# zhai-lw/L3AC

Measured on AMD Instinct MI355X. Metric: audio samples/sec encode+decode, 1kbps@16kHz, batch 256; indices bit-exact, higher is better.
Workload: dtype f32

## Files before the change

l3ac_amd/csrc/capi.hip:

```cpp
#include <algorithm>
#include <cmath>
#include <cstdarg>
#include <cstdlib>
#include <cstring>
#include <new>
#include <string>
#include <vector>

#include "network.hpp"
#include "kernels/split_bf16.hpp"

static thread_local std::string g_last_error;

void l3ac_set_error(const char* fmt, ...) {
    char buf[1024];
    va_list ap;
    va_start(ap, fmt);
    vsnprintf(buf, sizeof(buf), fmt, ap);
    va_end(ap);
    g_last_error = buf;
}

int l3ac_device_cu_count() {
    static std::atomic<int> cus[L3AC_MAX_DEVICES] = {};
// ... 97 lines not shown
template <class Map>
auto lookup(const Map& m, const char* name, const char* kind) -> decltype(m.begin()->second) {
    if (!name) {
        l3ac_set_error("null block name");
        return nullptr;
    }
    auto it = m.find(name);
    if (it == m.end()) {
        l3ac_set_error("no %s block named '%s'", kind, name);
        return nullptr;
    }
    return it->second;
}

struct Option {
    const char* name;
    int& (*field)(l3ac_ctx&);
    bool flag;
    int lo, hi, def;
    const char* env;
};
#define L3AC_FIELD(member) [](l3ac_ctx& c) -> int& { return c.member; }
const Option kOptions[] = {
    {"gemm_split", L3AC_FIELD(gemm_split), true, 0, 1, 1, "L3AC_GEMM_SPLIT"},
    {"head_pretanh", L3AC_FIELD(head_pretanh), true, 0, 1, 0, nullptr},
    {"narrow_ring", L3AC_FIELD(narrow_ring), false, 0, 2, 1, nullptr},
    {"wide_sliced", L3AC_FIELD(wide_sliced), false, 0, 2, 1, nullptr},
    {"unit_counter", L3AC_FIELD(unit_counter), false, 0, 3, 1, "L3AC_UNIT_COUNTER"},
    {"trans_coop", L3AC_FIELD(coop.enabled), true, 0, 1, 1, "L3AC_TRANS_COOP"},
    {"coop_timeout_ms", L3AC_FIELD(coop.timeout_ms), false, 1, 20000, 250, nullptr},
    {"down_fused", L3AC_FIELD(down_fused), false, 0, 2, 2, "L3AC_DOWN_FUSED"},
    {"gemm_w256", L3AC_FIELD(gemm_w256), false, 0, 2, 1, "L3AC_GEMM_W256"},
    {"unit_chunk_mb", L3AC_FIELD(unit_chunk_mb), false, 0, 65536, 192, "L3AC_UNIT_CHUNK_MB"},
};
#undef L3AC_FIELD

const Option* find_option(const char* name) {
    for (const Option& o : kOptions)
        if (std::strcmp(o.name, name) == 0) return &o;
    return nullptr;
}

int unknown_option(const char* who, const char* name) {
    std::string names;
    for (const Option& o : kOptions) names += std::string(names.empty() ? "" : ", ") + o.name;
    l3ac_set_error("%s: unknown option '%s' (%s; to set only: coop_release_claim, coop_test_fault)", who, name, names.c_str());
    return L3AC_EINVAL;
}

int initial_value(const Option& o) {
    const char* e = o.env ? std::getenv(o.env) : nullptr;
    return e ? std::atoi(e) : o.def;
}

int checked_value(const Option& o, int value) { return o.flag ? value != 0 : std::min(std::max(value, o.lo), o.hi); }

int set_checked(l3ac_ctx* ctx, const Option& o, int value, const char* who) {
    L3AC_REQUIRE(!(std::strcmp(o.name, "down_fused") == 0 && value == 1),
                 "%s: down_fused = 1 (the bf16x3 one-kernel down layers) was retired, DESIGN.md section 4; 2 (the default) is the one-kernel "
                 "form with the bits of 0, the GEMM + row kernel", who);
    o.field(*ctx) = checked_value(o, value);
    return L3AC_OK;
}

int ragged_plan(l3ac_ctx* ctx, hipStream_t s, RaggedPlan& p, int batch, int max_tok, const int32_t* n_tok, const int32_t* samples) {
    p.max_tok = max_tok;
// ... 282 lines not shown
                    const float* w_out, const float* b_out, float* q_feature, void* stream) {
    L3AC_REQUIRE(indices && levels && n_levels >= 1 && n_levels <= L3AC_MAX_LEVELS, "fsq_decode: bad arguments");
    FsqArgs f{};
    f.idx_in = indices; f.n = n; f.feat = feat; f.n_levels = n_levels;
    for (int d = 0; d < n_levels; ++d) f.levels[d] = levels[d];
    f.w_out = w_out; f.b_out = b_out; f.q_feature = q_feature;
    return launch_fsq((hipStream_t)stream, f);
}

int l3ac_fsq_copy_ceiling(const float* x, int64_t n, float* q_feature, int32_t* indices, float* level_indices, void* stream) {
    return launch_fsq_copy_ceiling((hipStream_t)stream, x, n, q_feature, indices, level_indices);
}
int l3ac_fsq_copy_ceiling_at(const float* x, int64_t n, float* q_feature, int32_t* indices, float* level_indices, int32_t blocks_per_cu, void* stream) {
    return launch_fsq_copy_ceiling((hipStream_t)stream, x, n, q_feature, indices, level_indices, blocks_per_cu);
}

int64_t l3ac_vq_argmin_scratch_bytes(int64_t n, int32_t k, int32_t form) {
    return (n > 0 && k > 0) ? (int64_t)vq_argmin_scratch_bytes(n, k, form) : 0;
}

int l3ac_vq_argmin(const float* queries, int64_t n, const float* codebook, int32_t k, int32_t dim, int32_t* out_idx,
                   void* scratch, int64_t scratch_bytes, int32_t form, void* stream) {
    L3AC_REQUIRE(queries && codebook && out_idx, "vq_argmin: null buffer");
    if (n == 0) return L3AC_OK;
    L3AC_REQUIRE(form == 0 || form == 1, "vq_argmin: form must be 0 (automatic) or 1 (direct-form scan)");
    L3AC_REQUIRE(scratch && k > 0 && scratch_bytes >= (int64_t)vq_argmin_scratch_bytes(n, k, form),
                 "vq_argmin: scratch of %lld bytes needed (l3ac_vq_argmin_scratch_bytes), %lld given",
                 (long long)(k > 0 ? vq_argmin_scratch_bytes(n, k, form) : 0), (long long)scratch_bytes);
    return launch_vq_argmin((hipStream_t)stream, queries, n, codebook, k, dim, scratch, out_idx, form);
}

int l3ac_op_first_block(l3ac_ctx* ctx, const float* audio, int32_t batch, int32_t samples, float* y, void* stream) {
    L3AC_ENTER_WS(ctx, stream);
    return launch_first_block((hipStream_t)stream, ctx->first, audio, samples, batch, samples, samples, y);
}

int l3ac_op_first_block_at(l3ac_ctx* ctx, const float* audio, int32_t batch, int32_t samples, int64_t audio_stride, int32_t frames,
                           float* y, void* stream) {
    L3AC_ENTER_WS(ctx, stream);
    L3AC_REQUIRE(audio && y && batch > 0, "op_first_block_at: bad arguments");
    L3AC_REQUIRE(samples > 0 && frames >= samples, "op_first_block_at: frames %d < samples %d, or samples <= 0", frames, samples);
    L3AC_REQUIRE(audio_stride >= samples, "op_first_block_at: stride %lld < samples %d", (long long)audio_stride, samples);
    return launch_first_block((hipStream_t)stream, ctx->first, audio, audio_stride, batch, samples, frames, y);
}

static int op_shape_ok(int batch, int frames) {
    L3AC_REQUIRE(frames <= L3AC_MAX_CLIP_FRAMES, "block entry: %d frames per clip, the limit is 2^31 - 65536 (32-bit frame numbers)", frames);
    L3AC_REQUIRE((int64_t)batch * frames < L3AC_MAX_ROWS, "block entry: batch * frames = %lld, the limit is 2^34 rows (32-bit tile numbers)",
                 (long long)batch * frames);
    return L3AC_OK;
}

#define L3AC_OP_SCRATCH(c_max)                                                                                    \
    L3AC_TRY(op_shape_ok(batch, frames));                                                                         \
    L3AC_TRY(workspace_ensure(ctx, (size_t)batch * frames * (c_max), (size_t)batch * frames * (c_max),           \
                              std::max((size_t)batch * frames * 4 * (c_max),                                      \
                                       (conv_unit_wide_scratch_bytes((c_max), (int64_t)batch * frames) + 3) / 4), \
                              (size_t)batch * frames * 4, (size_t)batch, (hipStream_t)stream))

int l3ac_op_conv_unit(l3ac_ctx* ctx, const char* block, const float* x, int32_t batch, int32_t frames, float* y,
                      void* stream) {
    L3AC_ENTER_WS(ctx, stream);
    const ConvUnitW* w = lookup(ctx->by_unit, block, "ConvUnit");
    if (!w) return L3AC_EINVAL;
    L3AC_TRY(conv_unit_shape_ok(ctx, *w, x == y, frames));
    L3AC_OP_SCRATCH(w->c);
    return run_conv_unit(ctx, (hipStream_t)stream, *w, x, y, batch, frames);
}

int l3ac_op_down_layer(l3ac_ctx* ctx, const char* block, const float* x, int32_t batch, int32_t frames, float* y,
                       void* stream) {
    L3AC_ENTER_WS(ctx, stream);
    const DownW* w = lookup(ctx->by_down, block, "down-layer");
    if (!w) return L3AC_EINVAL;
    L3AC_REQUIRE(x != y, "op_down_layer: x and y must not alias");
    return run_down(ctx, (hipStream_t)stream, *w, x, y, batch, frames);
// ... 165 lines not shown
        out[slot].ms_total += ms;
        out[slot].flops += r.flops;
        out[slot].bytes += r.bytes;
    }
    if (p->failed && rc == L3AC_OK) {
        l3ac_set_error("profile: event creation failed");
        rc = L3AC_EHIP;
    }
    delete p;
    if (n_out) *n_out = n;
    return rc;
}

int l3ac_gemm_f32(const float* a, int64_t lda, const float* w, const float* bias, float* c, int64_t ldc, int64_t m,
                  int32_t n, int32_t k, void* stream) {
    GemmArgs g{};
    g.a = a; g.lda = lda; g.w = w; g.ldw = k; g.c = c; g.ldc = ldc; g.m = m; g.n = n; g.k = k; g.bias = bias; g.epi = EPI_BIAS;
    return launch_gemm((hipStream_t)stream, g);
}

void l3ac_split3_host(const float* x, int64_t n, uint16_t* planes) {
    for (int64_t i = 0; i < n; ++i) {
        uint16_t pl[3];
        split3_host(x[i], pl);
        planes[i] = pl[0];
        planes[n + i] = pl[1];
        planes[2 * n + i] = pl[2];
    }
}

int l3ac_ctx_set_head_pretanh(l3ac_ctx* ctx, int32_t enable) { return l3ac_ctx_set_option(ctx, "head_pretanh", enable); }

int l3ac_op_snake(const float* x, float* y, int64_t rows, int32_t c, const float* alpha, int32_t mode, void* stream) {
    L3AC_REQUIRE(x && y && alpha && rows >= 0 && c > 0 && c % 4 == 0 && c <= 4096 && mode >= 0 && mode <= 4, "op_snake: bad arguments");
    hipStream_t s = (hipStream_t)stream;
    float* inv = nullptr;
    std::vector<float> ha((size_t)c), hi((size_t)c);
    L3AC_HIP_CHECK(hipMemcpyAsync(ha.data(), alpha, (size_t)c * sizeof(float), hipMemcpyDeviceToHost, s));
    L3AC_HIP_CHECK(hipStreamSynchronize(s));
    for (int i = 0; i < c; ++i) hi[i] = 1.0f / (ha[i] + 1e-8f);
    L3AC_HIP_CHECK(hipMalloc((void**)&inv, (size_t)c * sizeof(float)));
    int rc = L3AC_OK;
    if (hipMemcpyAsync(inv, hi.data(), (size_t)c * sizeof(float), hipMemcpyHostToDevice, s) != hipSuccess) {
        l3ac_set_error("op_snake: upload failed");
        rc = L3AC_EHIP;
    }
    if (rc == L3AC_OK) rc = launch_snake(s, x, y, rows, c, alpha, inv, mode);
    (void)hipStreamSynchronize(s);
    (void)hipFree(inv);
    return rc;
}

int l3ac_ctx_set_option(l3ac_ctx* ctx, const char* name, int32_t value) {
    L3AC_REQUIRE(ctx != nullptr && name != nullptr, "set_option: null argument");
    if (std::strcmp(name, "coop_release_claim") == 0) {
        trans_coop_release(ctx->coop);
        return L3AC_OK;
    }
    if (std::strcmp(name, "coop_test_fault") == 0) {
        ctx->coop.fault_part = value - 1;
        return L3AC_OK;
    }
    const Option* o = find_option(name);
    return o ? set_checked(ctx, *o, value, "set_option") : unknown_option("set_option", name);
}

int l3ac_ctx_get_option(const l3ac_ctx* ctx, const char* name, int32_t* out) {
// ... 35 lines not shown
```

l3ac_amd/csrc/kernels.hpp:

```cpp
#pragma once

#include "common.hpp"

enum GemmEpilogue : int {
    EPI_BIAS = 0,
    EPI_BIAS_RES = 1,
    EPI_SNAKE = 2,
    EPI_SNAKE_GRN = 3,
    EPI_GEGLU = 4,
};

struct GemmArgs {
    const float* a = nullptr;
    int64_t lda = 0;
    int taps = 1, dil = 1, cin = 0;
    int64_t frames = 0;
    const float* w = nullptr;
    int64_t ldw = 0;
    const unsigned char* w_img = nullptr;
    float* c = nullptr;
    int64_t ldc = 0;
    int64_t m = 0;
    int n = 0, k = 0;
    int epi = EPI_BIAS;
// ... 39 lines not shown
};
struct RowArgs {
    const float* x = nullptr;
    float* y = nullptr;
    int64_t batch = 0, frames_in = 0, frames_out = 0;
    int c = 0;
    int src = SRC_PLAIN, norm = NORM_NONE;
    const float* dw_w = nullptr;
    const float* dw_b = nullptr;
    int scale = 1;
    const float* yi = nullptr;
    const float* stats = nullptr;
    const float* in_w = nullptr;
    const float* in_b = nullptr;
    const float* gate_w = nullptr;
    const float* gate_b = nullptr;
    const float* nw = nullptr;
    const float* nb = nullptr;
    float eps = 0.f;
};
int launch_rows(hipStream_t s, const RowArgs& r);

int launch_snake(hipStream_t s, const float* x, float* y, int64_t rows, int c, const float* alpha,
                 const float* inv_alpha, int mode = 0);
int launch_geglu(hipStream_t s, const float* h, int64_t ldh, float* y, int64_t ldy, int64_t rows, int inner);
int launch_grn_sumsq(hipStream_t s, const float* h, int64_t batch, int64_t per_clip, float* sumsq);
int launch_grn_apply(hipStream_t s, float* h, int64_t batch, int64_t frames, int c, const float* sumsq,
                     const float* gamma, const float* beta, float* min_track = nullptr);

struct FirstBlockW {
    const float* tw;
    const float* tb;
    const float* w1;
    const float* b1;
    const float* w2;
    const float* b2;
    int d0;
};
struct RaggedClips {
    const int* n = nullptr;
    int mult = 1;
    const int* samples = nullptr;
};
int launch_first_block(hipStream_t s, const FirstBlockW& w, const float* audio, int64_t audio_stride, int batch,
                       int samples, int frames, float* y, const RaggedClips* rc = nullptr);

struct EnhanceW {
    const float* tw;
    const float* tb;
};
int launch_enhance_branches(hipStream_t s, const EnhanceW& w, const float* x, int batch, int frames, int c, float* yi,
                            const RaggedClips* rc = nullptr);
int launch_enhance_stats(hipStream_t s, float* yi, int batch, int frames, float* stats, const RaggedClips* rc = nullptr);

int launch_head(hipStream_t s, const float* x, int batch, int frames, int c, const float* w ,
                const float* b, float* audio, bool pretanh = false);

int launch_attention(hipStream_t s, const float* qkv, float* out, const float* bias_table ,
                     int batch, int frames, int heads, int dh, int window);

struct FsqArgs {
    const float* x = nullptr;
    int64_t n = 0;
    int feat = 0, n_levels = 0;
    int levels[L3AC_MAX_LEVELS] = {0};
    const float* w_in = nullptr;
    const float* b_in = nullptr;
    const float* w_out = nullptr;
    const float* b_out = nullptr;
    const int32_t* idx_in = nullptr;
    float* q_feature = nullptr;
    int32_t* indices = nullptr;
    float* level_indices = nullptr;
    float* latents = nullptr;
    bool act_in = false;
    int* bad_count = nullptr;
};
int launch_fsq(hipStream_t s, const FsqArgs& a);
// ... 47 lines not shown
```

l3ac_amd/csrc/kernels/device_math.hpp:

```cpp
#pragma once

#include <hip/hip_runtime.h>

constexpr float SIN2_ARG_MAX = 1.0e5f;

__device__ __forceinline__ float sin_squared(float u) {
    u = __builtin_amdgcn_fmed3f(u, -SIN2_ARG_MAX, SIN2_ARG_MAX);
    const float n = rintf(u * 0.636619772367581343f);
    float r = fmaf(n, -1.57079637050628662109375f, u);
    r = fmaf(n, 4.37113900018624283e-8f, r);
    const float z = r * r;
    float p = fmaf(z, -1.9515295891e-4f, 8.3321608736e-3f);
    p = fmaf(p, z, -1.6666654611e-1f);
    const float s = fmaf(p * z, r, r);
    const float s2 = s * s;
    return ((int)n & 1) ? 1.0f - s2 : s2;
}

__device__ __forceinline__ float snake_act(float h, float alpha, float inv_alpha) {
    return fmaf(inv_alpha, sin_squared(alpha * h), h);
}

typedef float f32x2 __attribute__((ext_vector_type(2)));
typedef int i32x2 __attribute__((ext_vector_type(2)));

__device__ __forceinline__ f32x2 sin_squared2(f32x2 u) {
    u.x = __builtin_amdgcn_fmed3f(u.x, -SIN2_ARG_MAX, SIN2_ARG_MAX);
    u.y = __builtin_amdgcn_fmed3f(u.y, -SIN2_ARG_MAX, SIN2_ARG_MAX);
    const f32x2 n = __builtin_elementwise_rint(u * 0.636619772367581343f);
    f32x2 r = __builtin_elementwise_fma(n, (f32x2)(-1.57079637050628662109375f), u);
    r = __builtin_elementwise_fma(n, (f32x2)(4.37113900018624283e-8f), r);
    const f32x2 z = r * r;
    f32x2 p = __builtin_elementwise_fma(z, (f32x2)(-1.9515295891e-4f), (f32x2)(8.3321608736e-3f));
    p = __builtin_elementwise_fma(p, z, (f32x2)(-1.6666654611e-1f));
    const f32x2 s = __builtin_elementwise_fma(p * z, r, r);
    const f32x2 c = __builtin_elementwise_fma(s * s, (f32x2)(-2.0f), (f32x2)(1.0f));
    const i32x2 cb = __builtin_bit_cast(i32x2, c) ^ (__builtin_convertvector(n, i32x2) << 31);
    return __builtin_elementwise_fma(__builtin_bit_cast(f32x2, cb), (f32x2)(-0.5f), (f32x2)(0.5f));
}

__device__ __forceinline__ f32x2 snake_act2(f32x2 h, f32x2 alpha, f32x2 inv_alpha) {
    return __builtin_elementwise_fma(inv_alpha, sin_squared2(alpha * h), h);
}

__device__ __forceinline__ float gelu_erf(float x) { return 0.5f * x * (1.0f + erff(x * 0.70710678118654752440f)); }
```

l3ac_amd/csrc/kernels/first_block.hip:

```cpp
#include "../kernels.hpp"
#include "device_math.hpp"

namespace {

constexpr int TILE = 256;
constexpr int HALO = 47;


template <int FT, int NT>
__device__ __forceinline__ void first_block_trends(const FirstBlockW& w, const float* __restrict__ clip, const int t0, const int samples, const int frames,
                                                   const int tid, const int f, float* xs, float* mbuf, float* pbuf, float (&h)[20]) {
    for (int i = tid; i < FT + 2 * HALO; i += NT) {
        const int u = t0 - HALO + i;
        xs[i] = (u >= 0 && u < samples) ? clip[u] : 0.f;
    }
    __syncthreads();
    {
#pragma unroll
        for (int o = 0; o < 4; ++o) {
            float acc = w.tb[o];
#pragma unroll
            for (int j = 0; j < 7; ++j) acc = fmaf(w.tw[o * 7 + j], xs[HALO + f + j - 3], acc);
            h[o] = acc;
        }
// ... 96 lines not shown
    const int b = blockIdx.y;
    const int t0 = blockIdx.x * FT;
    float h[20];
    first_block_trends<FT, 256>(w, audio + (int64_t)b * audio_stride, t0, RAGGED ? rs[b] : samples, RAGGED ? rn[b] * rmult : frames, tid, f,
                                xs, mbuf, pbuf, h);
#pragma unroll 4
    for (int oo = 0; oo < 20; ++oo) {
        const int o = 20 * part + oo;
        float s = w.b1[o];
#pragma unroll
        for (int i = 0; i < 20; ++i) s = fmaf(w.w1[o * 20 + i], h[i], s);
        gbuf[o][f] = gelu_erf(s);
    }
    __syncthreads();
    const int t = t0 + f;
    if (t >= frames) return;
    float out[DP];
#pragma unroll
    for (int d = 0; d < DP; ++d) out[d] = w.b2[DP * part + d];
#pragma unroll 8
    for (int o = 0; o < 80; ++o) {
        const float g = gbuf[o][f];
#pragma unroll
        for (int d = 0; d < DP; ++d) out[d] = fmaf(w.w2[o * D0 + DP * part + d], g, out[d]);
    }
    const float xv = xs[HALO + f];
#pragma unroll
    for (int d = 0; d < DP; ++d) out[d] = fmaf(w.w2[80 * D0 + DP * part + d], xv, out[d]);
    float* dst = y + ((int64_t)b * frames + t) * D0 + DP * part;
#pragma unroll
    for (int d = 0; d < DP; d += 2) *reinterpret_cast<float2*>(dst + d) = make_float2(out[d], out[d + 1]);
}

}

int launch_first_block(hipStream_t s, const FirstBlockW& w, const float* audio, int64_t audio_stride, int batch,
                       int samples, int frames, float* y, const RaggedClips* rc) {
    L3AC_REQUIRE(batch > 0 && batch <= 65535 && frames >= samples && samples > 0, "first_block: bad shape");
    L3AC_REQUIRE(frames <= L3AC_MAX_CLIP_FRAMES, "first_block: %d frames per clip, the limit is 2^31 - 65536 (32-bit frame numbers)", frames);
    const dim3 grid((unsigned)ceil_div64(frames, TILE), (unsigned)batch);
    const int* rn = rc ? rc->n : nullptr;
    const int* rs = rc ? rc->samples : nullptr;
    const int rmult = rc ? rc->mult : 1;
    ProfScope prof(s, rc ? "first_block_kernel<RAGGED>" : "first_block_kernel", 2.0 * (140.0 + 1600.0 + 81.0 * w.d0 + 164.0) * batch * frames,
                   4.0 * ((double)batch * samples + (double)batch * frames * w.d0));
    const dim3 grid_split((unsigned)ceil_div64(frames, 64), (unsigned)batch);
    const bool few = (int64_t)grid_split.x * grid_split.y <= 1024;
    switch (w.d0) {
#define L3AC_FB_CASE(D)                                                                                                       \
    case D:                                                                                                                   \
        if (rc && few)                                                                                                        \
            hipLaunchKernelGGL((first_block_split_kernel<D, true>), grid_split, dim3(256), 0, s, w, audio, audio_stride, samples,   \
                               frames, y, rn, rmult, rs);                                                                     \
        else if (rc)                                                                                                          \
            hipLaunchKernelGGL((first_block_kernel<D, 1, true>), grid, dim3(TILE), 0, s, w, audio, audio_stride, samples, frames, y, \
                               rn, rmult, rs);                                                                                \
        else if (few)                                                                                                         \
            hipLaunchKernelGGL((first_block_split_kernel<D, false>), grid_split, dim3(256), 0, s, w, audio, audio_stride, samples,  \
                               frames, y, rn, rmult, rs);                                                                     \
        else                                                                                                                  \
            hipLaunchKernelGGL((first_block_kernel<D, 1, false>), grid, dim3(TILE), 0, s, w, audio, audio_stride, samples, frames, y, \
                               rn, rmult, rs);                                                                                \
        break
        L3AC_FB_CASE(8);
        L3AC_FB_CASE(16);
        L3AC_FB_CASE(24);
        L3AC_FB_CASE(32);
#undef L3AC_FB_CASE
        default:
            l3ac_set_error("first_block: encoder_dims[0]=%d not in {8,16,24,32}", w.d0);
            return L3AC_EINVAL;
    }
    L3AC_LAUNCH_CHECK();
    return L3AC_OK;
}
```

l3ac_amd/csrc/kernels/rows.hip:

```cpp
#include "../kernels.hpp"
#include "device_math.hpp"
#include "lane_sums.hpp"

namespace {

constexpr int THREADS = 256;
constexpr int MAX_CH = 2;

__device__ __forceinline__ float group_sum(float v, int lpr, int pos) {
    if ((lpr & (lpr - 1)) == 0) return lanes_sum(v, lpr);
    for (int d = 1; d < lpr; d <<= 1) {
        const float o = __shfl_down(v, d, 64);
        v += pos + d < lpr ? o : 0.f;
    }
    return __shfl(v, (int)(threadIdx.x & 63) - pos, 64);
}

__device__ __forceinline__ float4 f4_fma(float4 a, float4 b, float4 c) {
    return make_float4(fmaf(a.x, b.x, c.x), fmaf(a.y, b.y, c.y), fmaf(a.z, b.z, c.z), fmaf(a.w, b.w, c.w));
}

template <int SRC, int NORM, class IDX, int LPR, int NCH>
__global__ __launch_bounds__(THREADS) void row_kernel(const RowArgs p, const int lpr_rt) {
    const int lpr = LPR ? LPR : lpr_rt;
// ... 223 lines not shown
                   4.0 * (in_elems + out_elems));
    const bool small = (double)r.batch * r.frames_in * r.c < 2147483648.0 && out_elems < 2147483648.0 && rows + blocks * 256 < ((int64_t)1 << 31);
#define L3AC_ROWS_LAUNCH(IDX_, LPR_)                                                                                             \
    do {                                                                                                                         \
        if (r.c <= 4 * lpr)                                                                                                      \
            hipLaunchKernelGGL((row_kernel<SRC, NORM, IDX_, LPR_, 1>), dim3((unsigned)blocks), dim3(THREADS), 0, s, r, lpr);     \
        else                                                                                                                     \
            hipLaunchKernelGGL((row_kernel<SRC, NORM, IDX_, LPR_, MAX_CH>), dim3((unsigned)blocks), dim3(THREADS), 0, s, r, lpr); \
    } while (0)
    if (!small) {
        L3AC_ROWS_LAUNCH(int64_t, 0);
    } else {
        switch (lpr) {
            case 6: L3AC_ROWS_LAUNCH(unsigned, 6); break;
            case 12: L3AC_ROWS_LAUNCH(unsigned, 12); break;
            case 32: L3AC_ROWS_LAUNCH(unsigned, 32); break;
            case 48: L3AC_ROWS_LAUNCH(unsigned, 48); break;
            case 64: L3AC_ROWS_LAUNCH(unsigned, 64); break;
            default: L3AC_ROWS_LAUNCH(unsigned, 0); break;
        }
    }
#undef L3AC_ROWS_LAUNCH
    L3AC_LAUNCH_CHECK();
    return L3AC_OK;
}

__global__ __launch_bounds__(THREADS) void snake_kernel(const float* __restrict__ x, float* __restrict__ y,
                                                       int64_t n4, int c4, const float* __restrict__ alpha,
                                                       const float* __restrict__ inv_alpha, const int mode) {
    for (int64_t i = (int64_t)blockIdx.x * THREADS + threadIdx.x; i < n4; i += (int64_t)gridDim.x * THREADS) {
        const int c0 = (int)(i % c4) << 2;
        const float4 v = reinterpret_cast<const float4*>(x)[i];
        float4 o;
        if (mode == 4) {
            o = make_float4(gelu_erf(v.x), gelu_erf(v.y), gelu_erf(v.z), gelu_erf(v.w));
        } else if (mode & 2) {
            if (mode & 1) {
                const f32x2 lo = sin_squared2(f32x2{v.x, v.y}), hi = sin_squared2(f32x2{v.z, v.w});
                o = make_float4(lo.x, lo.y, hi.x, hi.y);
            } else {
                o = make_float4(sin_squared(v.x), sin_squared(v.y), sin_squared(v.z), sin_squared(v.w));
            }
        } else {
            const float4 a = *reinterpret_cast<const float4*>(alpha + c0);
            const float4 ia = *reinterpret_cast<const float4*>(inv_alpha + c0);
            if (mode & 1) {
                const f32x2 lo = snake_act2(f32x2{v.x, v.y}, f32x2{a.x, a.y}, f32x2{ia.x, ia.y});
                const f32x2 hi = snake_act2(f32x2{v.z, v.w}, f32x2{a.z, a.w}, f32x2{ia.z, ia.w});
                o = make_float4(lo.x, lo.y, hi.x, hi.y);
            } else {
                o = make_float4(snake_act(v.x, a.x, ia.x), snake_act(v.y, a.y, ia.y), snake_act(v.z, a.z, ia.z),
                                snake_act(v.w, a.w, ia.w));
            }
        }
        reinterpret_cast<float4*>(y)[i] = o;
    }
}

__global__ __launch_bounds__(THREADS) void geglu_kernel(const float* __restrict__ h, int64_t ldh, float* __restrict__ y,
                                                       int64_t ldy, int64_t rows, int inner) {
    const int64_t total = rows * ldy;
    for (int64_t i = (int64_t)blockIdx.x * THREADS + threadIdx.x; i < total; i += (int64_t)gridDim.x * THREADS) {
        const int64_t r = i / ldy;
        const int j = (int)(i % ldy);
        float o = 0.f;
        if (j < inner) o = h[r * ldh + j] * gelu_erf(h[r * ldh + inner + j]);
        y[i] = o;
// ... 151 lines not shown
```

l3ac_amd/csrc/network.hip:

```cpp
#include "network.hpp"

#include <algorithm>
#include <cmath>
#include <cstring>
#include <functional>

namespace {

constexpr int HEADS = 6;

struct Builder {
    l3ac_ctx* ctx = nullptr;
    std::unordered_map<std::string, const l3ac_tensor*> map;
    std::vector<float> host;
    float* dev = nullptr;
    size_t cap = 0;
    std::string err;
    struct Image { size_t bytes; std::function<void(unsigned char*)> write; const unsigned char** target; };
    std::vector<Image> images;
    bool trans_stacks = false;
    const float* host_of(const float* d) const { return host.data() + (d - dev); }

    void image(std::vector<unsigned char> img, const unsigned char** target) {
        const size_t bytes = img.size();
// ... 33 lines not shown
    const float* copy(const std::string& name, int64_t numel) {
        const float* src = find(name, numel);
        const float* d = nullptr;
        float* h = alloc((size_t)numel, &d);
        if (src && d) std::memcpy(h, src, (size_t)numel * sizeof(float));
        return d;
    }
    const float* conv(const std::string& name, int co, int ci, int k) {
        const float* src = find(name, (int64_t)co * ci * k);
        const float* d = nullptr;
        float* h = alloc((size_t)co * ci * k, &d);
        if (src && d)
            for (int o = 0; o < co; ++o)
                for (int c = 0; c < ci; ++c)
                    for (int j = 0; j < k; ++j) h[((size_t)o * k + j) * ci + c] = src[((size_t)o * ci + c) * k + j];
        return d;
    }
    const float* dwconv(const std::string& name, int c) {
        const float* src = find(name, (int64_t)c * 7);
        const float* d = nullptr;
        float* h = alloc((size_t)c * 7, &d);
        if (src && d)
            for (int ch = 0; ch < c; ++ch)
                for (int j = 0; j < 7; ++j) h[(size_t)j * c + ch] = src[(size_t)ch * 7 + j];
        return d;
    }
    const float* transposed(const std::string& name, int n, int k) {
        const float* src = find(name, (int64_t)n * k);
        const float* d = nullptr;
        float* h = alloc((size_t)k * n, &d);
        if (src && d)
            for (int o = 0; o < n; ++o)
                for (int i = 0; i < k; ++i) h[(size_t)i * n + o] = src[(size_t)o * k + i];
        return d;
    }
    const float* ff_value_gate(const std::string& name, int ffi, int dim, int ff_n) {
        const float* src = find(name, (int64_t)2 * ffi * dim);
        const float* d = nullptr;
        float* h = alloc((size_t)ff_n * dim, &d);
        if (src && d)
            for (int j = 0; j < ffi; ++j) {
                const int jb = j / 32, r = j % 32;
                std::memcpy(h + (size_t)(64 * jb + r) * dim, src + (size_t)j * dim, dim * sizeof(float));
                std::memcpy(h + (size_t)(64 * jb + 32 + r) * dim, src + (size_t)(ffi + j) * dim, dim * sizeof(float));
            }
        return d;
    }
    const float* ff_padded(const std::string& name, int dim, int ffi, int ff_pad) {
        const float* src = find(name, (int64_t)dim * ffi);
        const float* d = nullptr;
        float* h = alloc((size_t)dim * ff_pad, &d);
        if (src && d)
            for (int o = 0; o < dim; ++o) std::memcpy(h + (size_t)o * ff_pad, src + (size_t)o * ffi, ffi * sizeof(float));
        return d;
    }
    void trend(const std::string& p, int n, int co, const float** tw, const float** tb) {
        float* hw = alloc((size_t)n * co * 7, tw);
        float* hb = alloc((size_t)n * co, tb);
        for (int i = 0; i < n; ++i) {
            const float* w = find(p + ".blocks." + std::to_string(i) + ".1.weight", co * 7);
            const float* bb = find(p + ".blocks." + std::to_string(i) + ".1.bias", co);
            if (w && bb && hw && hb) {
                std::memcpy(hw + (size_t)i * co * 7, w, (size_t)co * 7 * sizeof(float));
                std::memcpy(hb + (size_t)i * co, bb, co * sizeof(float));
            }
        }
// ... 13 lines not shown
const float* build_bias_table(Builder& b, const std::string& prefix, int dim, int window) {
    const int hdim = dim / 2;
    const float* w0 = b.find(prefix + ".mlp.0.weight", hdim);
    const float* b0 = b.find(prefix + ".mlp.0.bias", hdim);
    const float* w2 = b.find(prefix + ".mlp.2.weight", (int64_t)hdim * hdim);
    const float* b2 = b.find(prefix + ".mlp.2.bias", hdim);
    const float* w4 = b.find(prefix + ".mlp.4.weight", (int64_t)HEADS * hdim);
    const float* b4 = b.find(prefix + ".mlp.4.bias", HEADS);
    const float* d = nullptr;
    float* h = b.alloc((size_t)HEADS * 2 * window, &d);
    if (!(w0 && b0 && w2 && b2 && w4 && b4 && d)) return d;
    std::vector<float> h1(hdim), h2(hdim);
    for (int dist = 0; dist < 2 * window; ++dist) {
        for (int i = 0; i < hdim; ++i) h1[i] = silu(w0[i] * (float)dist + b0[i]);
        for (int i = 0; i < hdim; ++i) {
            float s = b2[i];
            for (int j = 0; j < hdim; ++j) s += w2[(size_t)i * hdim + j] * h1[j];
            h2[i] = silu(s);
        }
        for (int hd = 0; hd < HEADS; ++hd) {
            float s = b4[hd];
            for (int j = 0; j < hdim; ++j) s += w4[(size_t)hd * hdim + j] * h2[j];
            h[(size_t)hd * 2 * window + dist] = s;
        }
    }
    return d;
}


void build_first_block(Builder& b, FirstBlockW& f, const std::string& p, int d0) {
    b.trend(p, 5, 4, &f.tw, &f.tb);
    f.d0 = d0;
    f.w1 = b.copy(p + ".conv_1.weight", 80 * 20);
    f.b1 = b.copy(p + ".conv_1.bias", 80);
    f.w2 = b.transposed(p + ".conv_2.weight", d0, 81);
    f.b2 = b.copy(p + ".conv_2.bias", d0);
}

void build_conv_unit(Builder& b, ConvUnitW& u, const std::string& p, int c) {
    u.c = c;
    u.dw_w = b.dwconv(p + ".dw_conv.weight", c);
    u.dw_b = b.copy(p + ".dw_conv.bias", c);
    u.ln_w = b.copy(p + ".norm.weight", c);
    u.ln_b = b.copy(p + ".norm.bias", c);
    u.w1 = b.gemm(b.copy(p + ".pw_conv1.weight", (int64_t)4 * c * c), 4 * c, c);
    u.b1 = b.copy(p + ".pw_conv1.bias", 4 * c);
    u.alpha = b.copy(p + ".act.alpha", 4 * c);
    u.inv_alpha = b.inv_alpha(p + ".act.alpha", 4 * c);
    u.gamma = b.copy(p + ".grn.gamma", 4 * c);
    u.beta = b.copy(p + ".grn.beta", 4 * c);
    u.w2 = b.gemm(b.copy(p + ".pw_conv2.weight", (int64_t)4 * c * c), c, 4 * c);
    u.b2 = b.copy(p + ".pw_conv2.bias", c);
    if (b.err.empty()) {
        if (conv_unit_wide_supported(c)) {
            b.image(conv_unit_wide_image(b.host_of(u.w1), b.host_of(u.w2), c), &u.wide_img);
        } else if (conv_unit_fused_supported(c)) {
            b.image(conv_unit_w1_image(b.host_of(u.w1), c), &u.w1_img);
            b.image(conv_unit_w2_image(b.host_of(u.w2), c), &u.w2_img);
            if (conv_unit_ring_supported(c)) b.image(conv_unit_ring_image(b.host_of(u.w1), b.host_of(u.w2), c), &u.ring_img);
        }
    }
    b.ctx->by_unit[p] = &u;
}

void build_down(Builder& b, DownW& d, const std::string& p, int cin, int cout, int stride, bool norm) {
    d.cin = cin;
// ... 669 lines not shown
        GemmArgs g{};
        g.a = ws.a; g.lda = dim; g.w = l.wqkv; g.ldw = dim; g.c = ws.h; g.ldc = 3 * ctx->inner; g.m = rows; g.n = 3 * ctx->inner; g.k = dim;
        g.epi = EPI_BIAS;
        L3AC_TRY(gemm_on_route(ctx, s, g));
        L3AC_TRY(launch_attention(s, ws.h, ws.a, w.bias_table, batch, frames, HEADS, ctx->dim_head, w.window));
        GemmArgs go{};
        go.a = ws.a; go.lda = ctx->inner; go.w = l.wout; go.ldw = ctx->inner; go.c = x; go.ldc = dim; go.m = rows; go.n = dim; go.k = ctx->inner;
        go.epi = EPI_BIAS_RES; go.res = x; go.ldres = dim;
        L3AC_TRY(gemm_on_route(ctx, s, go));
        r.nw = l.ln2w; r.nb = l.ln2b;
        L3AC_TRY(launch_rows(s, r));
        GemmArgs f1{};
        f1.a = ws.a; f1.lda = dim; f1.w = l.wff1; f1.ldw = dim; f1.c = ws.h; f1.ldc = ctx->ff_pad; f1.m = rows; f1.n = ctx->ff_n; f1.k = dim;
        f1.epi = EPI_GEGLU; f1.n_out = ctx->ff_inner;
        L3AC_TRY(gemm_on_route(ctx, s, f1));
        GemmArgs f2{};
        f2.a = ws.h; f2.lda = ctx->ff_pad; f2.w = l.wff2; f2.ldw = ctx->ff_pad; f2.c = x; f2.ldc = dim; f2.m = rows; f2.n = dim; f2.k = ctx->ff_pad;
        f2.epi = EPI_BIAS_RES; f2.res = x; f2.ldres = dim;
        L3AC_TRY(gemm_on_route(ctx, s, f2));
    }
    return L3AC_OK;
}

static inline void swap_bufs(float** a, float** b) {
    float* t = *a;
    *a = *b;
    *b = t;
}

int run_encoder(l3ac_ctx* ctx, hipStream_t s, const float* audio, int64_t audio_stride, int batch, int samples,
                int frames, float** cur, float** alt) {
    const l3ac_config& c = ctx->cfg;
    const RaggedClips rc = ctx->rag ? ctx->rag->clips(frames) : RaggedClips{};
    L3AC_TRY(launch_first_block(s, ctx->first, audio, audio_stride, batch, samples, frames, *cur, ctx->rag ? &rc : nullptr));
    int f = frames;
    for (int i = 0; i < c.n_enc; ++i) {
        L3AC_TRY(run_conv_units(ctx, s, ctx->enc_units[i], cur, alt, batch, f));
        if (i + 1 < c.n_enc) {
            L3AC_TRY(run_down(ctx, s, ctx->enc_down[i], *cur, *alt, batch, f));
            swap_bufs(cur, alt);
            f /= c.compress_rates[i];
        }
    }
    L3AC_TRY(rag_mask(ctx, s, *cur, batch, f, c.enc_dims[c.n_enc - 1], 1));
    L3AC_TRY(run_conv_k3(ctx, s, ctx->enc_out, *cur, *alt, batch, f));
    swap_bufs(cur, alt);
    return L3AC_OK;
}

int run_en_encoder(l3ac_ctx* ctx, hipStream_t s, int batch, int frames, float** cur, float** alt, int* n_tok) {
    if (ctx->en_enc.size() == 2) {
        L3AC_TRY(local_trans_step(ctx, s, ctx->en_enc[0], cur, alt, batch, frames));
        L3AC_TRY(run_down(ctx, s, ctx->en_down, *cur, *alt, batch, frames));
        swap_bufs(cur, alt);
        frames /= ctx->en_down.stride;
        L3AC_TRY(local_trans_step(ctx, s, ctx->en_enc[1], cur, alt, batch, frames));
    } else {
        L3AC_TRY(local_trans_step(ctx, s, ctx->en_enc[0], cur, alt, batch, frames));
    }
    *n_tok = frames;
    return L3AC_OK;
}

int run_en_decoder(l3ac_ctx* ctx, hipStream_t s, int batch, int n_tok, float** cur, float** alt, int* frames) {
    L3AC_TRY(local_trans_step(ctx, s, ctx->en_dec[0], cur, alt, batch, n_tok));
    int f = n_tok;
    if (ctx->en_dec.size() == 2) {
// ... 33 lines not shown
```

l3ac_amd/csrc/network.hpp:

```cpp
#pragma once

#include <map>
#include <string>
#include <unordered_map>
#include <vector>

#include "kernels.hpp"

struct ConvUnitW {
    int c = 0;
    const float *dw_w, *dw_b, *ln_w, *ln_b, *w1, *b1, *alpha, *inv_alpha, *gamma, *beta, *w2, *b2;
    const unsigned char *w1_img = nullptr, *w2_img = nullptr;
    const unsigned char* wide_img = nullptr;
    const unsigned char* ring_img = nullptr;
};
struct DownW {
    int cin = 0, cout = 0, stride = 1;
    const float *w, *b, *nw = nullptr, *nb = nullptr;
    const unsigned char* exact_img = nullptr;
};
struct ConvK3W {
    int cin = 0, cout = 0;
    const float *w, *b;
};
// ... 44 lines not shown
    float *x0 = nullptr, *x1 = nullptr, *a = nullptr, *h = nullptr, *yi = nullptr, *stats = nullptr, *sumsq = nullptr;
    int* plan = nullptr;
    size_t x_cap = 0, a_cap = 0, h_cap = 0, yi_cap = 0, b_cap = 0;
    size_t bytes() const { return (2 * x_cap + a_cap + h_cap + yi_cap + 12 * b_cap) * sizeof(float); }
};

struct RaggedPlan {
    static constexpr int plan_ints() { return 3; }
    int max_tok = 0;
    std::vector<int> n_tok;
    std::vector<int> order;
    const int* n_dev = nullptr;
    const int* samples_dev = nullptr;
    const int* order_dev = nullptr;
    RaggedClips clips(int frames) const { return RaggedClips{n_dev, frames / max_tok, samples_dev}; }
};

struct l3ac_ctx {
    l3ac_config cfg{};
    int device = 0;
    int hop = 0, enc_rate = 1, dim_head = 0, inner = 0, ff_inner = 0, ff_pad = 0, ff_n = 0;
    float* arena = nullptr;
    size_t arena_floats = 0;
    unsigned char* img_arena = nullptr;
    size_t img_bytes = 0;
    std::unordered_map<const float*, const unsigned char*> split_img;
    int gemm_split, head_pretanh;
    int unit_counter;
    int wide_sliced;
    int narrow_ring;
    int down_fused;
    int gemm_w256;
    int unit_chunk_mb;
    const unsigned char* img(const float* w) const {
        if (!gemm_split) return nullptr;
        auto it = split_img.find(w);
        return it == split_img.end() ? nullptr : it->second;
    }

    FirstBlockW first{};
    std::vector<std::vector<ConvUnitW>> enc_units;
    std::vector<DownW> enc_down;
    ConvK3W enc_out{};
    std::vector<LocalTransW> en_enc;
    DownW en_down{};
    std::vector<LocalTransW> en_dec;
    const float *q_win = nullptr, *q_bin = nullptr, *q_wout = nullptr, *q_bout = nullptr;
    ConvK3W dec_in{};
    std::vector<std::vector<ConvUnitW>> dec_units;
    std::vector<EnhW> dec_enh;
    std::vector<UpW> dec_up;
    std::vector<LegacyW> legacy;
    HeadW head{};

    std::map<std::string, const ConvUnitW*> by_unit;
    std::map<std::string, const DownW*> by_down;
    std::map<std::string, const ConvK3W*> by_k3;
    std::map<std::string, const EnhW*> by_enh;
    std::map<std::string, const UpW*> by_up;
    std::map<std::string, const LocalTransW*> by_trans;

    Workspace ws;
    TransCoopState coop;
    int* bad_index_count = nullptr;
    int* wide_counters = nullptr;
    float* grn_min_sumsq = nullptr;
// ... 74 lines not shown
```

Before: 307.9 million.

## Add packed two-lane FMA stem kernels with fast small-argument GELU polynomial

```diff
diff --git a/l3ac_amd/csrc/capi.hip b/l3ac_amd/csrc/capi.hip
--- a/l3ac_amd/csrc/capi.hip
+++ b/l3ac_amd/csrc/capi.hip
@@ -153,6 +153,7 @@
     {"down_fused", L3AC_FIELD(down_fused), false, 0, 2, 2, "L3AC_DOWN_FUSED"},
     {"gemm_w256", L3AC_FIELD(gemm_w256), false, 0, 2, 1, "L3AC_GEMM_W256"},
     {"unit_chunk_mb", L3AC_FIELD(unit_chunk_mb), false, 0, 65536, 192, "L3AC_UNIT_CHUNK_MB"},
+    {"stem_packed", L3AC_FIELD(stem_packed), true, 0, 1, 1, nullptr},
 };
 #undef L3AC_FIELD
 
@@ -501,7 +502,7 @@
 
 int l3ac_op_first_block(l3ac_ctx* ctx, const float* audio, int32_t batch, int32_t samples, float* y, void* stream) {
     L3AC_ENTER_WS(ctx, stream);
-    return launch_first_block((hipStream_t)stream, ctx->first, audio, samples, batch, samples, samples, y);
+    return launch_first_block((hipStream_t)stream, ctx->first, audio, samples, batch, samples, samples, y, ctx->stem_packed != 0);
 }
 
 int l3ac_op_first_block_at(l3ac_ctx* ctx, const float* audio, int32_t batch, int32_t samples, int64_t audio_stride, int32_t frames,
@@ -510,7 +511,7 @@
     L3AC_REQUIRE(audio && y && batch > 0, "op_first_block_at: bad arguments");
     L3AC_REQUIRE(samples > 0 && frames >= samples, "op_first_block_at: frames %d < samples %d, or samples <= 0", frames, samples);
     L3AC_REQUIRE(audio_stride >= samples, "op_first_block_at: stride %lld < samples %d", (long long)audio_stride, samples);
-    return launch_first_block((hipStream_t)stream, ctx->first, audio, audio_stride, batch, samples, frames, y);
+    return launch_first_block((hipStream_t)stream, ctx->first, audio, audio_stride, batch, samples, frames, y, ctx->stem_packed != 0);
 }
 
 static int op_shape_ok(int batch, int frames) {
@@ -742,7 +743,7 @@
 int l3ac_ctx_set_head_pretanh(l3ac_ctx* ctx, int32_t enable) { return l3ac_ctx_set_option(ctx, "head_pretanh", enable); }
 
 int l3ac_op_snake(const float* x, float* y, int64_t rows, int32_t c, const float* alpha, int32_t mode, void* stream) {
-    L3AC_REQUIRE(x && y && alpha && rows >= 0 && c > 0 && c % 4 == 0 && c <= 4096 && mode >= 0 && mode <= 4, "op_snake: bad arguments");
+    L3AC_REQUIRE(x && y && alpha && rows >= 0 && c > 0 && c % 4 == 0 && c <= 4096 && mode >= 0 && mode <= 5, "op_snake: bad arguments");
     hipStream_t s = (hipStream_t)stream;
     float* inv = nullptr;
     std::vector<float> ha((size_t)c), hi((size_t)c);
diff --git a/l3ac_amd/csrc/kernels.hpp b/l3ac_amd/csrc/kernels.hpp
--- a/l3ac_amd/csrc/kernels.hpp
+++ b/l3ac_amd/csrc/kernels.hpp
@@ -95,6 +95,7 @@
     const float* tw;
     const float* tb;
     const float* w1;
+    const float* w1p;
     const float* b1;
     const float* w2;
     const float* b2;
@@ -106,7 +107,7 @@
     const int* samples = nullptr;
 };
 int launch_first_block(hipStream_t s, const FirstBlockW& w, const float* audio, int64_t audio_stride, int batch,
-                       int samples, int frames, float* y, const RaggedClips* rc = nullptr);
+                       int samples, int frames, float* y, bool packed, const RaggedClips* rc = nullptr);
 
 struct EnhanceW {
     const float* tw;
diff --git a/l3ac_amd/csrc/kernels/device_math.hpp b/l3ac_amd/csrc/kernels/device_math.hpp
--- a/l3ac_amd/csrc/kernels/device_math.hpp
+++ b/l3ac_amd/csrc/kernels/device_math.hpp
@@ -44,3 +44,41 @@
 }
 
 __device__ __forceinline__ float gelu_erf(float x) { return 0.5f * x * (1.0f + erff(x * 0.70710678118654752440f)); }
+
+typedef float f32x4 __attribute__((ext_vector_type(4)));
+
+template <class V>
+__device__ __forceinline__ V gelu_erf_small(const V x, const V a) {
+    const V t = a * a;
+    V p = __builtin_elementwise_fma(t, (V)(-0x1.268bc2p-11f), (V)(0x1.420828p-8f));
+    p = __builtin_elementwise_fma(t, p, (V)(-0x1.b5937p-6f));
+    p = __builtin_elementwise_fma(t, p, (V)(0x1.ce077cp-4f));
+    p = __builtin_elementwise_fma(t, p, (V)(-0x1.81266p-2f));
+    p = __builtin_elementwise_fma(t, p, (V)(0x1.06eba0p-3f));
+    const V e = __builtin_elementwise_fma(a, p, a);
+    return (0.5f * x) * (1.0f + e);
+}
+
+__device__ __forceinline__ f32x2 gelu_erf2(f32x2 x) {
+    const f32x2 a = x * 0.70710678118654752440f;
+    const bool large = !(__builtin_fabsf(a.x) < 1.0f) || !(__builtin_fabsf(a.y) < 1.0f);
+    if (__builtin_amdgcn_ballot_w64(large) != 0) return f32x2{gelu_erf(x.x), gelu_erf(x.y)};
+    return gelu_erf_small(x, a);
+}
+
+__device__ __forceinline__ void gelu_erf2x2(f32x2& x0, f32x2& x1) {
+    f32x4 x = __builtin_shufflevector(x0, x1, 0, 1, 2, 3);
+    const f32x4 a = x * 0.70710678118654752440f;
+    const bool large = !(__builtin_fabsf(a.x) < 1.0f) || !(__builtin_fabsf(a.y) < 1.0f) || !(__builtin_fabsf(a.z) < 1.0f) ||
+                       !(__builtin_fabsf(a.w) < 1.0f);
+    if (__builtin_amdgcn_ballot_w64(large) != 0) {
+#pragma unroll 1
+        for (int e = 0; e < 4; ++e) x = f32x4{x.y, x.z, x.w, gelu_erf(x.x)};
+        x0 = __builtin_shufflevector(x, x, 0, 1);
+        x1 = __builtin_shufflevector(x, x, 2, 3);
+        return;
+    }
+    const f32x4 g = gelu_erf_small(x, a);
+    x0 = __builtin_shufflevector(g, g, 0, 1);
+    x1 = __builtin_shufflevector(g, g, 2, 3);
+}
diff --git a/l3ac_amd/csrc/kernels/first_block.hip b/l3ac_amd/csrc/kernels/first_block.hip
--- a/l3ac_amd/csrc/kernels/first_block.hip
+++ b/l3ac_amd/csrc/kernels/first_block.hip
@@ -152,10 +152,137 @@
     for (int d = 0; d < DP; d += 2) *reinterpret_cast<float2*>(dst + d) = make_float2(out[d], out[d + 1]);
 }
 
+
+template <int I>
+__device__ __forceinline__ f32x2 splat_half(const f32x2 v) {
+    return __builtin_shufflevector(v, v, I, I);
+}
+
+__device__ __forceinline__ void stem_pack_h(const float (&h)[20], f32x2 (&hp)[10]) {
+#pragma unroll
+    for (int k = 0; k < 10; ++k) hp[k] = f32x2{h[2 * k], h[2 * k + 1]};
+}
+
+__device__ __forceinline__ void stem_hidden_pairs(const FirstBlockW& w, const int p, f32x2 (&hp)[10], f32x2& g0, f32x2& g1) {
+#pragma unroll
+    for (int k = 0; k < 10; ++k) asm("" : "+v"(hp[k]) : "s"(p));
+    const f32x2* __restrict__ wa = reinterpret_cast<const f32x2*>(w.w1p) + p * 20;
+    const f32x2* __restrict__ wb = wa + 20;
+    f32x2 s0 = reinterpret_cast<const f32x2*>(w.b1)[p], s1 = reinterpret_cast<const f32x2*>(w.b1)[p + 1];
+#pragma unroll
+    for (int k = 0; k < 10; ++k) {
+        s0 = __builtin_elementwise_fma(wa[2 * k], splat_half<0>(hp[k]), s0);
+        s1 = __builtin_elementwise_fma(wb[2 * k], splat_half<0>(hp[k]), s1);
+        s0 = __builtin_elementwise_fma(wa[2 * k + 1], splat_half<1>(hp[k]), s0);
+        s1 = __builtin_elementwise_fma(wb[2 * k + 1], splat_half<1>(hp[k]), s1);
+    }
+    gelu_erf2x2(s0, s1);
+    g0 = s0;
+    g1 = s1;
+}
+
+template <int D0, bool RAGGED>
+__global__ __launch_bounds__(TILE) void first_block_packed_kernel(const FirstBlockW w, const float* __restrict__ audio,
+                                                                 int64_t audio_stride, int samples, int frames,
+                                                                 float* __restrict__ y, const int* __restrict__ rn, int rmult,
+                                                                 const int* __restrict__ rs) {
+    constexpr int DH = D0 / 2;
+    __shared__ float xs[TILE + 2 * HALO];
+    __shared__ float mbuf[TILE + 6 + 44];
+    __shared__ float pbuf[TILE + 6];
+
+    const int tid = threadIdx.x;
+    const int b = blockIdx.y;
+    const int t0 = blockIdx.x * TILE;
+    float h[20];
+    first_block_trends<TILE, TILE>(w, audio + (int64_t)b * audio_stride, t0, RAGGED ? rs[b] : samples, RAGGED ? rn[b] * rmult : frames,
+                                   tid, tid, xs, mbuf, pbuf, h);
+
+    const int t = t0 + tid;
+    if (t >= frames) return;
+
+    f32x2 hp[10];
+    stem_pack_h(h, hp);
+    const f32x2* __restrict__ w2 = reinterpret_cast<const f32x2*>(w.w2);
+    f32x2 out[DH];
+#pragma unroll
+    for (int d = 0; d < DH; ++d) out[d] = reinterpret_cast<const f32x2*>(w.b2)[d];
+#pragma unroll 1
+    for (int p = 0; p < 40; p += 2) {
+        f32x2 g[2];
+        stem_hidden_pairs(w, p, hp, g[0], g[1]);
+#pragma unroll
+        for (int e = 0; e < 2; ++e) {
+#pragma unroll
+            for (int d = 0; d < DH; ++d) out[d] = __builtin_elementwise_fma(w2[(2 * (p + e)) * DH + d], splat_half<0>(g[e]), out[d]);
+#pragma unroll
+            for (int d = 0; d < DH; ++d) out[d] = __builtin_elementwise_fma(w2[(2 * (p + e) + 1) * DH + d], splat_half<1>(g[e]), out[d]);
+        }
+    }
+    const float xv = xs[HALO + tid];
+#pragma unroll
+    for (int d = 0; d < DH; ++d) out[d] = __builtin_elementwise_fma(w2[80 * DH + d], f32x2{xv, xv}, out[d]);
+
+    float* dst = y + ((int64_t)b * frames + t) * D0;
+#pragma unroll
+    for (int d = 0; d < DH; d += 2) *reinterpret_cast<float4*>(dst + 2 * d) = make_float4(out[d].x, out[d].y, out[d + 1].x, out[d + 1].y);
+}
+
+template <int D0, bool RAGGED>
+__global__ __launch_bounds__(256) void first_block_split_packed_kernel(const FirstBlockW w, const float* __restrict__ audio, int64_t audio_stride,
+                                                                       int samples, int frames, float* __restrict__ y, const int* __restrict__ rn,
+                                                                       int rmult, const int* __restrict__ rs) {
+    constexpr int FT = 64, DP = D0 / 4;
+    static_assert(D0 % 8 == 0, "two floats per store");
+    __shared__ float xs[FT + 2 * HALO];
+    __shared__ float mbuf[FT + 6 + 44];
+    __shared__ float pbuf[FT + 6];
+    __shared__ float gbuf[80][FT];
+    const int tid = threadIdx.x;
+    const int f = tid & 63;
+    const int part = __builtin_amdgcn_readfirstlane(tid >> 6);
+    const int b = blockIdx.y;
+    const int t0 = blockIdx.x * FT;
+    float h[20];
+    first_block_trends<FT, 256>(w, audio + (int64_t)b * audio_stride, t0, RAGGED ? rs[b] : samples, RAGGED ? rn[b] * rmult : frames, tid, f,
+                                xs, mbuf, pbuf, h);
+    f32x2 hp[10];
+    stem_pack_h(h, hp);
+#pragma unroll 1
+    for (int pp = 0; pp < 10; pp += 2) {
+        const int p = 10 * part + pp;
+        f32x2 g[2];
+        stem_hidden_pairs(w, p, hp, g[0], g[1]);
+#pragma unroll
+        for (int e = 0; e < 2; ++e) {
+            gbuf[2 * (p + e)][f] = g[e].x;
+            gbuf[2 * (p + e) + 1][f] = g[e].y;
+        }
+    }
+    __syncthreads();
+    const int t = t0 + f;
+    if (t >= frames) return;
+    float out[DP];
+#pragma unroll
+    for (int d = 0; d < DP; ++d) out[d] = w.b2[DP * part + d];
+#pragma unroll 8
+    for (int o = 0; o < 80; ++o) {
+        const float g = gbuf[o][f];
+#pragma unroll
+        for (int d = 0; d < DP; ++d) out[d] = fmaf(w.w2[o * D0 + DP * part + d], g, out[d]);
+    }
+    const float xv = xs[HALO + f];
+#pragma unroll
+    for (int d = 0; d < DP; ++d) out[d] = fmaf(w.w2[80 * D0 + DP * part + d], xv, out[d]);
+    float* dst = y + ((int64_t)b * frames + t) * D0 + DP * part;
+#pragma unroll
+    for (int d = 0; d < DP; d += 2) *reinterpret_cast<float2*>(dst + d) = make_float2(out[d], out[d + 1]);
+}
+
 }
 
 int launch_first_block(hipStream_t s, const FirstBlockW& w, const float* audio, int64_t audio_stride, int batch,
-                       int samples, int frames, float* y, const RaggedClips* rc) {
+                       int samples, int frames, float* y, bool packed, const RaggedClips* rc) {
     L3AC_REQUIRE(batch > 0 && batch <= 65535 && frames >= samples && samples > 0, "first_block: bad shape");
     L3AC_REQUIRE(frames <= L3AC_MAX_CLIP_FRAMES, "first_block: %d frames per clip, the limit is 2^31 - 65536 (32-bit frame numbers)", frames);
     const dim3 grid((unsigned)ceil_div64(frames, TILE), (unsigned)batch);
@@ -167,26 +294,32 @@
     const dim3 grid_split((unsigned)ceil_div64(frames, 64), (unsigned)batch);
     const bool few = (int64_t)grid_split.x * grid_split.y <= 1024;
     switch (w.d0) {
-#define L3AC_FB_CASE(D)                                                                                                       \
-    case D:                                                                                                                   \
-        if (rc && few)                                                                                                        \
-            hipLaunchKernelGGL((first_block_split_kernel<D, true>), grid_split, dim3(256), 0, s, w, audio, audio_stride, samples,   \
-                               frames, y, rn, rmult, rs);                                                                     \
-        else if (rc)                                                                                                          \
-            hipLaunchKernelGGL((first_block_kernel<D, 1, true>), grid, dim3(TILE), 0, s, w, audio, audio_stride, samples, frames, y, \
-                               rn, rmult, rs);                                                                                \
-        else if (few)                                                                                                         \
-            hipLaunchKernelGGL((first_block_split_kernel<D, false>), grid_split, dim3(256), 0, s, w, audio, audio_stride, samples,  \
-                               frames, y, rn, rmult, rs);                                                                     \
-        else                                                                                                                  \
-            hipLaunchKernelGGL((first_block_kernel<D, 1, false>), grid, dim3(TILE), 0, s, w, audio, audio_stride, samples, frames, y, \
-                               rn, rmult, rs);                                                                                \
+#define L3AC_FB_LAUNCH(KERNEL, GRID, BLOCK) \
+    hipLaunchKernelGGL(KERNEL, GRID, dim3(BLOCK), 0, s, w, audio, audio_stride, samples, frames, y, rn, rmult, rs)
+#define L3AC_FB_FORMS(D, RAG)                                                                       \
+    if (few && packed)                                                                              \
+        L3AC_FB_LAUNCH((first_block_split_packed_kernel<D, RAG>), grid_split, 256);                 \
+    else if (few)                                                                                   \
+        L3AC_FB_LAUNCH((first_block_split_kernel<D, RAG>), grid_split, 256);                        \
+    else if (packed)                                                                                \
+        L3AC_FB_LAUNCH((first_block_packed_kernel<D, RAG>), grid, TILE);                            \
+    else                                                                                            \
+        L3AC_FB_LAUNCH((first_block_kernel<D, 1, RAG>), grid, TILE)
+#define L3AC_FB_CASE(D)              \
+    case D:                          \
+        if (rc) {                    \
+            L3AC_FB_FORMS(D, true);  \
+        } else {                     \
+            L3AC_FB_FORMS(D, false); \
+        }                            \
         break
         L3AC_FB_CASE(8);
         L3AC_FB_CASE(16);
         L3AC_FB_CASE(24);
         L3AC_FB_CASE(32);
 #undef L3AC_FB_CASE
+#undef L3AC_FB_FORMS
+#undef L3AC_FB_LAUNCH
         default:
             l3ac_set_error("first_block: encoder_dims[0]=%d not in {8,16,24,32}", w.d0);
             return L3AC_EINVAL;
diff --git a/l3ac_amd/csrc/kernels/rows.hip b/l3ac_amd/csrc/kernels/rows.hip
--- a/l3ac_amd/csrc/kernels/rows.hip
+++ b/l3ac_amd/csrc/kernels/rows.hip
@@ -279,7 +279,10 @@
         const int c0 = (int)(i % c4) << 2;
         const float4 v = reinterpret_cast<const float4*>(x)[i];
         float4 o;
-        if (mode == 4) {
+        if (mode == 5) {
+            const f32x2 lo = gelu_erf2(f32x2{v.x, v.y}), hi = gelu_erf2(f32x2{v.z, v.w});
+            o = make_float4(lo.x, lo.y, hi.x, hi.y);
+        } else if (mode == 4) {
             o = make_float4(gelu_erf(v.x), gelu_erf(v.y), gelu_erf(v.z), gelu_erf(v.w));
         } else if (mode & 2) {
             if (mode & 1) {
diff --git a/l3ac_amd/csrc/network.hip b/l3ac_amd/csrc/network.hip
--- a/l3ac_amd/csrc/network.hip
+++ b/l3ac_amd/csrc/network.hip
@@ -89,6 +89,15 @@
         if (src && d)
             for (int o = 0; o < n; ++o)
                 for (int i = 0; i < k; ++i) h[(size_t)i * n + o] = src[(size_t)o * k + i];
+        return d;
+    }
+    const float* pair_interleaved(const std::string& name, int n, int k) {
+        const float* src = find(name, (int64_t)n * k);
+        const float* d = nullptr;
+        float* h = alloc((size_t)n * k, &d);
+        if (src && d)
+            for (int o = 0; o < n; ++o)
+                for (int i = 0; i < k; ++i) h[((size_t)(o / 2) * k + i) * 2 + o % 2] = src[(size_t)o * k + i];
         return d;
     }
     const float* ff_value_gate(const std::string& name, int ffi, int dim, int ff_n) {
@@ -168,6 +177,7 @@
     b.trend(p, 5, 4, &f.tw, &f.tb);
     f.d0 = d0;
     f.w1 = b.copy(p + ".conv_1.weight", 80 * 20);
+    f.w1p = b.pair_interleaved(p + ".conv_1.weight", 80, 20);
     f.b1 = b.copy(p + ".conv_1.bias", 80);
     f.w2 = b.transposed(p + ".conv_2.weight", d0, 81);
     f.b2 = b.copy(p + ".conv_2.bias", d0);
@@ -903,7 +913,7 @@
                 int frames, float** cur, float** alt) {
     const l3ac_config& c = ctx->cfg;
     const RaggedClips rc = ctx->rag ? ctx->rag->clips(frames) : RaggedClips{};
-    L3AC_TRY(launch_first_block(s, ctx->first, audio, audio_stride, batch, samples, frames, *cur, ctx->rag ? &rc : nullptr));
+    L3AC_TRY(launch_first_block(s, ctx->first, audio, audio_stride, batch, samples, frames, *cur, ctx->stem_packed != 0, ctx->rag ? &rc : nullptr));
     int f = frames;
     for (int i = 0; i < c.n_enc; ++i) {
         L3AC_TRY(run_conv_units(ctx, s, ctx->enc_units[i], cur, alt, batch, f));
diff --git a/l3ac_amd/csrc/network.hpp b/l3ac_amd/csrc/network.hpp
--- a/l3ac_amd/csrc/network.hpp
+++ b/l3ac_amd/csrc/network.hpp
@@ -100,6 +100,7 @@
     int down_fused;
     int gemm_w256;
     int unit_chunk_mb;
+    int stem_packed;
     const unsigned char* img(const float* w) const {
         if (!gemm_split) return nullptr;
         auto it = split_img.find(w);
```

Measured after the change: 309.0 million, median of 6. No clear change (+0.4%).
